# ylsung/vl-merging

Measured on AMD Instinct MI355X. Metric: VL samples/sec (fwd+bwd) base_vl 384^2 at 1/2/4/8 GPUs; merge GB/s vs HBM peak, higher is better.
Workload: dtype bf16

## Files before the change

### vl-merging_amd/csrc/rowops.hip

```cpp
#include "vlm_common.h"

#ifndef ROW_NT
#define ROW_NT true
#endif
#define ROW_THREADS 256
#define ROW_WAVES 4

template <int MAXU, bool IN_BF16, bool NT = false>
__device__ __forceinline__ void load_row(const void* base, size_t row, int ld, int D, int lane, f32x4 (&v)[MAXU]) {
#pragma unroll
  for (int u = 0; u < MAXU; ++u) {
    const int c = lane * 4 + 256 * u;
    if (c < D) {
      if (IN_BF16) {
        const bf16x4* q = reinterpret_cast<const bf16x4*>(reinterpret_cast<const bf16_t*>(base) + row * ld + c);
        const bf16x4 h = NT ? __builtin_nontemporal_load(q) : *q;
        v[u] = (f32x4){(float)h[0], (float)h[1], (float)h[2], (float)h[3]};
      } else {
        const f32x4* q = reinterpret_cast<const f32x4*>(reinterpret_cast<const float*>(base) + row * ld + c);
        v[u] = NT ? __builtin_nontemporal_load(q) : *q;
      }
    } else {
      v[u] = (f32x4){0.f, 0.f, 0.f, 0.f};
    }
  }
}

template <int MAXU>
__device__ __forceinline__ void load_vec(const float* p, int D, int lane, f32x4 (&v)[MAXU], float fill) {
#pragma unroll
  for (int u = 0; u < MAXU; ++u) {
    const int c = lane * 4 + 256 * u;
    v[u] = (c < D && p) ? *reinterpret_cast<const f32x4*>(p + c) : (f32x4){fill, fill, fill, fill};
// ... 35 lines not shown
    if (stats && lane == 0) {
      stats[2 * row] = mean;
      stats[2 * row + 1] = rstd;
    }
#pragma unroll
    for (int u = 0; u < MAXU; ++u) {
      const int c = lane * 4 + 256 * u;
      if (c < D) {
        f32x4 o;
#pragma unroll
        for (int r = 0; r < 4; ++r) o[r] = (v[u][r] - mean) * rstd * g[u][r] + b[u][r];
        if (OUT_F32) {
          *reinterpret_cast<f32x4*>(reinterpret_cast<float*>(y) + row * ldy + c) = o;
        } else {
          bf16x4 h = {(bf16_t)o[0], (bf16_t)o[1], (bf16_t)o[2], (bf16_t)o[3]};
          *reinterpret_cast<bf16x4*>(reinterpret_cast<bf16_t*>(y) + row * ldy + c) = h;
        }
      }
    }
  }
}

struct ls_t {
  const bf16_t* y;
  int ldy;
  const float* gamma;
  const float* row_scale;
  bf16_t* dy;
  int lddy;
  float* dgamma;
  float* dbias;
  float* partials;
};
template <int MAXU, bool DY_BF16, int SCALE = 0>
__global__ __launch_bounds__(ROW_THREADS, MAXU <= 3 ? (SCALE ? 3 : 4) : 2) void ln_bwd_kernel(const void* __restrict__ dy, int lddy,
                                                             const float* __restrict__ x, int ldx,
                                                             const float* __restrict__ stats,
                                                             const float* __restrict__ gamma, int M, int D,
                                                             const float* __restrict__ dres, int lddres,
                                                             float* __restrict__ dx, int lddx,
                                                             float* __restrict__ dgamma, float* __restrict__ dbeta,
                                                             float* __restrict__ partials, const ls_t ls) {
  __shared__ float red[ROW_WAVES][SCALE ? 4 : 2][MAXU * 256];
  const int lane = threadIdx.x & 63, wave = threadIdx.x >> 6;
  f32x4 g[SCALE ? 1 : MAXU], ag[MAXU], ab[MAXU];
  f32x4 g2[1], ag2[SCALE == 1 ? MAXU : 1], ab2[SCALE ? MAXU : 1];
  if (SCALE) g[0] = (f32x4){1.f, 1.f, 1.f, 1.f};
  else load_vec<SCALE ? 1 : MAXU>(gamma, D, lane, g, 1.0f);
#pragma unroll
  for (int u = 0; u < MAXU; ++u) ag[u] = ab[u] = (f32x4){0.f, 0.f, 0.f, 0.f};
#pragma unroll
  for (int u = 0; u < (SCALE ? MAXU : 1); ++u) ab2[u] = (f32x4){0.f, 0.f, 0.f, 0.f};
#pragma unroll
  for (int u = 0; u < (SCALE == 1 ? MAXU : 1); ++u) ag2[u] = (f32x4){0.f, 0.f, 0.f, 0.f};
  const float invD = 1.0f / (float)D;
  for (size_t row = (size_t)blockIdx.x * ROW_WAVES + wave; row < (size_t)M; row += (size_t)gridDim.x * ROW_WAVES) {
    f32x4 v[MAXU], d[MAXU], rs[MAXU];
    load_row<MAXU, false, ROW_NT>(x, row, ldx, D, lane, v);
    load_row<MAXU, DY_BF16>(dy, row, lddy, D, lane, d);
    if (dres) load_row<MAXU, false, ROW_NT>(dres, row, lddres, D, lane, rs);
    f32x4 yy[SCALE == 1 ? MAXU : 1];
    float srow = 1.0f;
    if (SCALE) {
      if (SCALE == 1) load_row<SCALE == 1 ? MAXU : 1, true, ROW_NT>(ls.y, row, ls.ldy, D, lane, yy);
      if (ls.row_scale) srow = ls.row_scale[row];
    }
    const float mean = stats[2 * row], rstd = stats[2 * row + 1];
    float s1 = 0.f, s2 = 0.f;
#pragma unroll
    for (int u = 0; u < MAXU; ++u) {
      const int c = lane * 4 + 256 * u;
      if (c < D) {
        const f32x4 gu = (SCALE && gamma) ? *reinterpret_cast<const f32x4*>(gamma + c) : g[SCALE ? 0 : u];
#pragma unroll
        for (int r = 0; r < 4; ++r) {
          const float xh = (v[u][r] - mean) * rstd;
          const float gg = d[u][r] * gu[r];
          s1 += gg;
          s2 += gg * xh;
          ag[u][r] += d[u][r] * xh;
          ab[u][r] += d[u][r];
          v[u][r] = xh;
          d[u][r] = gg;
        }
      }
    }
    const float m1 = wave_sum(s1) * invD, m2 = wave_sum(s2) * invD;
#pragma unroll
    for (int u = 0; u < MAXU; ++u) {
      const int c = lane * 4 + 256 * u;
      if (c < D) {
        f32x4 o;
#pragma unroll
        for (int r = 0; r < 4; ++r) o[r] = rstd * (d[u][r] - m1 - v[u][r] * m2);
        if (dres) o += rs[u];
        *reinterpret_cast<f32x4*>(dx + row * lddx + c) = o;
        if (SCALE) {
          const int c2 = lane * 4 + 256 * u;
          g2[0] = (SCALE == 1 && ls.gamma) ? *reinterpret_cast<const f32x4*>(ls.gamma + c2) : (f32x4){1.f, 1.f, 1.f, 1.f};
          bf16x4 h;
#pragma unroll
          for (int r = 0; r < 4; ++r) {
            const float sd = srow * o[r];
            const float q = sd * g2[0][r];
            if (SCALE == 1) ag2[SCALE == 1 ? u : 0][r] += sd * yy[SCALE == 1 ? u : 0][r];
            h[r] = (bf16_t)q;
            ab2[u][r] += (float)h[r];
          }
          *reinterpret_cast<bf16x4*>(ls.dy + row * ls.lddy + c) = h;
        }
      }
    }
  }
  if (SCALE) {
#pragma unroll
    for (int u = 0; u < (SCALE ? MAXU : 1); ++u)
#pragma unroll
      for (int r = 0; r < 4; ++r) {
        red[wave][SCALE ? 2 : 0][u * 256 + lane * 4 + r] = SCALE == 1 ? ag2[SCALE == 1 ? u : 0][r] : 0.f;
        red[wave][SCALE ? 3 : 1][u * 256 + lane * 4 + r] = ab2[u][r];
      }
  }
  if (dgamma || dbeta || SCALE) {
#pragma unroll
    for (int u = 0; u < MAXU; ++u)
#pragma unroll
      for (int r = 0; r < 4; ++r) {
        red[wave][0][u * 256 + lane * 4 + r] = ag[u][r];
        red[wave][1][u * 256 + lane * 4 + r] = ab[u][r];
      }
    __syncthreads();
    for (int c = threadIdx.x; c < D; c += ROW_THREADS) {
      float sg = 0.f, sb = 0.f;
#pragma unroll
      for (int w = 0; w < ROW_WAVES; ++w) {
        sg += red[w][0][c];
        sb += red[w][1][c];
      }
      if (partials) {
        partials[((size_t)blockIdx.x * 2 + 0) * D + c] = sg;
        partials[((size_t)blockIdx.x * 2 + 1) * D + c] = sb;
      } else {
        if (dgamma) atomicAdd(dgamma + c, sg);
        if (dbeta) atomicAdd(dbeta + c, sb);
      }
      if (SCALE) {
        float tg = 0.f, tb = 0.f;
#pragma unroll
        for (int w = 0; w < ROW_WAVES; ++w) {
          tg += red[w][SCALE ? 2 : 0][c];
          tb += red[w][SCALE ? 3 : 1][c];
        }
        if (ls.partials) {
          ls.partials[((size_t)blockIdx.x * 2 + 0) * D + c] = tg;
          ls.partials[((size_t)blockIdx.x * 2 + 1) * D + c] = tb;
        } else {
          if (ls.dgamma) atomicAdd(ls.dgamma + c, tg);
          if (ls.dbias) atomicAdd(ls.dbias + c, tb);
        }
      }
    }
  }
}

__global__ __launch_bounds__(256) void colreduce_kernel(const float* __restrict__ partials, int nblocks, int D,
                                                        float* __restrict__ out0, float* __restrict__ out1) {
  const int i = blockIdx.x * 256 + threadIdx.x;
  if (i >= 2 * D) return;
  const int which = i / D, c = i - which * D;
  float* out = which ? out1 : out0;
  if (!out) return;
  const int per = (nblocks + gridDim.y - 1) / gridDim.y;
  const int b0 = blockIdx.y * per, b1 = min(nblocks, b0 + per);
  float s0 = 0.f, s1 = 0.f;
  int b = b0;
  for (; b + 1 < b1; b += 2) {
    s0 += partials[((size_t)(b + 0) * 2 + which) * D + c];
    s1 += partials[((size_t)(b + 1) * 2 + which) * D + c];
  }
  if (b < b1) s0 += partials[((size_t)b * 2 + which) * D + c];
  if (b0 < b1) atomicAdd(out + c, s0 + s1);
}

struct fold_jobs_t {
  vlm_fold_job_t j[VLM_MAX_FOLD_JOBS];
};
__global__ __launch_bounds__(256) void colreduce_batch_kernel(const fold_jobs_t jobs) {
  const vlm_fold_job_t job = jobs.j[blockIdx.z];
  const int D = job.D, i = blockIdx.x * 256 + threadIdx.x;
  if (i >= 2 * D) return;
  const int which = i / D, c = i - which * D;
  float* out = which ? job.out1 : job.out0;
  if (!out) return;
  const int per = (job.nblocks + gridDim.y - 1) / gridDim.y;
// ... 117 lines not shown
  int want = (M + ROW_WAVES - 1) / ROW_WAVES;
  int cap = cus * 8;
  return want < cap ? (want > 0 ? want : 1) : cap;
}

extern "C" int vlm_layernorm_fwd(const float* x, int ldx, int M, int D, const float* gamma, const float* beta,
                                 float eps, void* y, int ldy, int y_is_f32, float* stats, void* stream) {
  if (M == 0) return VLM_OK;
  if (!x || !y || M < 0 || D <= 0 || (D & 3) || (ldx & 3) || (ldy & 3)) return VLM_ERR_ARG;
  if (D > 1024) return VLM_ERR_UNSUPPORTED;
  dim3 grid(row_grid(M)), block(ROW_THREADS);
  hipStream_t s = (hipStream_t)stream;
#define LN_FWD(U, F) hipLaunchKernelGGL((ln_fwd_kernel<U, F>), grid, block, 0, s, x, ldx, M, D, gamma, beta, eps, y, ldy, stats)
  if (D <= 256) { if (y_is_f32) LN_FWD(1, true); else LN_FWD(1, false); }
  else if (D <= 768) { if (y_is_f32) LN_FWD(3, true); else LN_FWD(3, false); }
  else { if (y_is_f32) LN_FWD(4, true); else LN_FWD(4, false); }
#undef LN_FWD
  VLM_CHECK_LAUNCH();
  return VLM_OK;
}

static int layernorm_bwd_impl(const void* dy, int lddy, int dy_is_f32, const float* x, int ldx,
                              const float* stats, const float* gamma, int M, int D, const float* dres,
                              int lddres, float* dx, int lddx, float* dgamma, float* dbeta, float* workspace,
                              size_t workspace_bytes, int* deferred_blocks, void* stream, const vlm_layerscale_t* sc) {
  if (M == 0) return VLM_OK;
  if (!dy || !x || !stats || !dx || M < 0 || D <= 0 || (D & 3) || (ldx & 3) || (lddy & 3) || (lddx & 3) ||
      (dres && (lddres & 3)))
    return VLM_ERR_ARG;
  if (D > 1024) return VLM_ERR_UNSUPPORTED;
  int g = row_grid(M);
  const int resident = (D <= 768 ? 4 : 2) * (vlm_device_cus() > 0 ? vlm_device_cus() : 256);
  if (g > resident) g = resident;
  if (sc && D <= 768 && g > resident * 3 / 4) g = resident * 3 / 4;
  float* part = (workspace && workspace_bytes >= (size_t)g * 2 * D * sizeof(float) && (dgamma || dbeta)) ? workspace : nullptr;
  dim3 grid(g), block(ROW_THREADS);
  hipStream_t s = (hipStream_t)stream;
  ls_t ls = {};
  if (sc) {
    if (!sc->dy || (sc->y && (sc->ldy & 3)) || (sc->lddy & 3)) return VLM_ERR_ARG;
    if (!sc->y && (sc->gamma || sc->dgamma)) return VLM_ERR_ARG;
    const bool want = sc->dgamma || sc->dbias;
    float* part2 = (sc->workspace && sc->workspace_bytes >= (size_t)g * 2 * D * sizeof(float) && want) ? sc->workspace : nullptr;
    if (deferred_blocks && want && !part2) return VLM_ERR_ARG;
    ls.y = reinterpret_cast<const bf16_t*>(sc->y); ls.ldy = sc->ldy; ls.gamma = sc->gamma; ls.row_scale = sc->row_scale;
    ls.dy = reinterpret_cast<bf16_t*>(sc->dy); ls.lddy = sc->lddy; ls.dgamma = sc->dgamma; ls.dbias = sc->dbias; ls.partials = part2;
  }
#define LN_BWD(U, B)                                                                                                             \
  do {                                                                                                                           \
    if (sc && sc->y) hipLaunchKernelGGL((ln_bwd_kernel<U, B, 1>), grid, block, 0, s, dy, lddy, x, ldx, stats, gamma, M, D, dres, lddres, dx, lddx, dgamma, dbeta, part, ls); \
    else if (sc) hipLaunchKernelGGL((ln_bwd_kernel<U, B, 2>), grid, block, 0, s, dy, lddy, x, ldx, stats, gamma, M, D, dres, lddres, dx, lddx, dgamma, dbeta, part, ls); \
    else hipLaunchKernelGGL((ln_bwd_kernel<U, B, 0>), grid, block, 0, s, dy, lddy, x, ldx, stats, gamma, M, D, dres, lddres, dx, lddx, dgamma, dbeta, part, ls); \
  } while (0)
  if (D <= 256) { if (dy_is_f32) LN_BWD(1, false); else LN_BWD(1, true); }
  else if (D <= 768) { if (dy_is_f32) LN_BWD(3, false); else LN_BWD(3, true); }
  else { if (dy_is_f32) LN_BWD(4, false); else LN_BWD(4, true); }
#undef LN_BWD
  VLM_CHECK_LAUNCH();
  if (deferred_blocks) {
    if (!part && (dgamma || dbeta)) return VLM_ERR_ARG;
    *deferred_blocks = (part || ls.partials) ? g : 0;
  } else {
    if (part) {
      hipLaunchKernelGGL(colreduce_kernel, dim3((2 * D + 255) / 256, 32), dim3(256), 0, s, part, g, D, dgamma, dbeta);
      VLM_CHECK_LAUNCH();
    }
    if (ls.partials) {
      hipLaunchKernelGGL(colreduce_kernel, dim3((2 * D + 255) / 256, 32), dim3(256), 0, s, ls.partials, g, D, ls.dgamma, ls.dbias);
      VLM_CHECK_LAUNCH();
    }
  }
  return VLM_OK;
}

extern "C" int vlm_layernorm_bwd(const void* dy, int lddy, int dy_is_f32, const float* x, int ldx,
                                 const float* stats, const float* gamma, int M, int D, const float* dres,
                                 int lddres, float* dx, int lddx, float* dgamma, float* dbeta, float* workspace,
                                 size_t workspace_bytes, int* deferred_blocks, void* stream) {
  return layernorm_bwd_impl(dy, lddy, dy_is_f32, x, ldx, stats, gamma, M, D, dres, lddres, dx, lddx, dgamma, dbeta, workspace,
                            workspace_bytes, deferred_blocks, stream, nullptr);
}

extern "C" int vlm_layernorm_bwd_scale(const void* dy, int lddy, int dy_is_f32, const float* x, int ldx,
                                       const float* stats, const float* gamma, int M, int D, const float* dres,
                                       int lddres, float* dx, int lddx, float* dgamma, float* dbeta, float* workspace,
// ... 53 lines not shown
```

### vl-merging_amd/engine.py

```python
import itertools
import math
import os
import weakref
from typing import List, Optional

import torch

from . import _lib as L
from . import ops

BF16, F32 = torch.bfloat16, torch.float32
ALIGN = 64


def _touch_hook(p):
    p._vlm_flat.touched.add(p._vlm_name)


def touch(*params):
    for p in params:
        if p is not None:
            f = getattr(p, "_vlm_flat", None)
            if f is not None:
                f.touched.add(p._vlm_name)
# ... 488 lines not shown


def _fb(b):
    return b._vlm_folded if b is not None else None


def _rb(b):
    return b._vlm_raw if b is not None else None


def _arm_layerscale_finish(flat):
    if getattr(flat, "_ls_armed", False):
        return
    flat._ls_armed = True

    def done():
        flat._ls_armed = False
        flat.finish_layerscale()
        sync_wgrad()

    torch.autograd.Variable._execution_engine.queue_callback(done)


def _ln2_bwd_scale1(dln, x1, st2, e, dx1, dx2, y1, g1, rs1, dy1, fold):
    sgamma, dsgamma, dsbias = (None, None, _rb(e.projb)) if y1 is None else (g1, g1.grad, e.projb.grad)
    if x1.shape[1] <= 768:
        ops.layernorm_bwd_scale(dln, x1, st2, e.n2w, dx1, dx2, e.n2w.grad, e.n2b.grad, y=y1, sgamma=sgamma, row_scale=rs1,
                                sdy=dy1, dsgamma=dsgamma, dsbias=dsbias, fold=fold)
    else:
        ops.layernorm_bwd(dln, x1, st2, e.n2w, dx1, dres=dx2, dgamma=e.n2w.grad, dbeta=e.n2b.grad, fold=fold)
        ops.layerscale_bwd(dx1, y1, sgamma, rs1, dy1, dsgamma, dsbias, fold=fold)


class _BlockFn(torch.autograd.Function):

    @staticmethod
    def forward(ctx, x, bias_t, plan: BlockPlan, pc: PassCtx, training: bool, hook):
        M, D = x.shape
        dev = x.device
        H = pc.H
        Fdim = plan.ranges[0][2].fc1w.shape[0]
        x = x.contiguous()
        ln1 = torch.empty(M, D, device=dev, dtype=BF16)
        st1 = torch.empty(M, 2, device=dev, dtype=F32)
        qkv = torch.empty(M, 3 * D, device=dev, dtype=BF16)
        rs1 = pc.drop_path_rows(plan.drop_prob, training, dev)
        rs2 = pc.drop_path_rows(plan.drop_prob, training, dev)
        rg = plan.ranges
        for r0, r1, e in rg:
            ops.layernorm_fwd(x[r0:r1], e.n1w, e.n1b, plan.eps, ln1[r0:r1], st1[r0:r1])
        _gemm_rows(ln1, [(r0, r1, w16(e.qkvw), _qkv_bias(e), None) for r0, r1, e in rg], qkv)
        o = torch.empty(M, D, device=dev, dtype=BF16)
        lse = torch.empty(H, M, device=dev, dtype=F32)
        rp = pc.relpos
        ops.attention_fwd(qkv, o, lse, pc.seq, H, bias_t=bias_t, head_row0=plan.layer * H,
                          rel_index=rp.index if rp is not None else None,
                          rel_index_t=rp.index_t if rp is not None else None, keep0=pc.keep0, keep1=pc.keep1,
                          mode=plan.mode, bias_dense=rp.dense_for(pc.seq, plan.mode) if rp is not None else None)
        x1 = torch.empty(M, D, device=dev, dtype=F32)
        folded = _folded(plan.ranges)
        y1 = torch.empty(M, D, device=dev, dtype=BF16) if not folded else None
        ln2 = torch.empty(M, D, device=dev, dtype=BF16)
        st2 = torch.empty(M, 2, device=dev, dtype=F32)
        h = torch.empty(M, Fdim, device=dev, dtype=BF16)
        a = torch.empty(M, Fdim, device=dev, dtype=BF16)
        x2 = torch.empty(M, D, device=dev, dtype=F32)
        y2 = torch.empty(M, D, device=dev, dtype=BF16) if not folded else None
        cs1, cs2 = (None, None) if folded else (plan.gamma1, plan.gamma2)
        pb = (lambda e: _fb(e.projb)) if folded else (lambda e: e.projb)
        fb2 = (lambda e: _fb(e.fc2b)) if folded else (lambda e: e.fc2b)
        _gemm_rows(o, [(r0, r1, w16(e.projw), pb(e), None) for r0, r1, e in rg], x1, col_scale=cs1, row_scale=rs1,
                   residual=x, aux=y1)
        for r0, r1, e in rg:
            ops.layernorm_fwd(x1[r0:r1], e.n2w, e.n2b, plan.eps, ln2[r0:r1], st2[r0:r1])
        _gemm_rows(ln2, [(r0, r1, w16(e.fc1w), e.fc1b, None) for r0, r1, e in rg], a, act=L.ACT_GELU_DERIV, aux=h)
        _gemm_rows(a, [(r0, r1, w16(e.fc2w), fb2(e), None) for r0, r1, e in rg], x2, col_scale=cs2, row_scale=rs2,
                   residual=x1, aux=y2)
        if pc.gram is not None:
            for r0, r1, e in plan.ranges:
                gn = e.gram_names
                if gn.get("qkv") or gn.get("fc1"):
                    t32 = torch.empty(r1 - r0, D, device=dev, dtype=F32)
                    st = torch.empty(r1 - r0, 2, device=dev, dtype=F32)
                    if gn.get("qkv"):
                        ops.layernorm_fwd(x[r0:r1], e.n1w, e.n1b, plan.eps, t32, st)
                        pc.gram.add(gn.get("qkv"), t32)
                    if gn.get("fc1"):
                        ops.layernorm_fwd(x1[r0:r1], e.n2w, e.n2b, plan.eps, t32, st)
                        pc.gram.add(gn.get("fc1"), t32)
                pc.gram.add(gn.get("proj"), o[r0:r1])
                pc.gram.add(gn.get("fc2"), a[r0:r1])
        ctx.plan, ctx.pc, ctx.hook = plan, pc, hook
        ctx.has_bias = bias_t is not None
        ctx.folded = folded
        ctx.save_for_backward(x, st1, ln1, qkv, o, lse, y1 if y1 is not None else x.new_empty(0), x1, st2, ln2, h, a,
                              y2 if y2 is not None else x.new_empty(0),
                              rs1 if rs1 is not None else x.new_empty(0), rs2 if rs2 is not None else x.new_empty(0),
                              bias_t if bias_t is not None else x.new_empty(0))
        return x2

    @staticmethod
    def backward(ctx, dx2):
        plan, pc = ctx.plan, ctx.pc
        x, st1, ln1, qkv, o, lse, y1, x1, st2, ln2, h, a, y2, rs1, rs2, bias_t = ctx.saved_tensors
        rs1 = rs1 if rs1.numel() else None
        rs2 = rs2 if rs2.numel() else None
        bias_t = bias_t if ctx.has_bias else None
        M, D = x.shape
        dev = x.device
        H = pc.H
        Fdim = h.shape[1]
        dx2 = dx2.contiguous()
        g1, g2 = plan.gamma1, plan.gamma2
        folded = ctx.folded
        if folded:
            y1 = y2 = None
            flat = plan.ranges[0][2].projw._vlm_flat
            _arm_layerscale_finish(flat)
        wg = (lambda w: w._vlm_raw) if folded else (lambda w: w.grad)
        touch(g1, g2)
        for _, _, e in plan.ranges:
            _touch_expert(e)
        dy2 = torch.empty(M, D, device=dev, dtype=BF16)
        dy1 = torch.empty(M, D, device=dev, dtype=BF16)
        dh = torch.empty(M, Fdim, device=dev, dtype=BF16)
        dln = torch.empty(M, D, device=dev, dtype=BF16)
        dx1 = torch.empty(M, D, device=dev, dtype=F32)
        fold = ops.FoldBatch(dev, D)
        rg = plan.ranges
        do = torch.empty(M, D, device=dev, dtype=BF16)
        for r0, r1, e in rg:
            rr = slice(r0, r1)
            if folded:
                ops.layerscale_bwd(dx2[rr], None, None, rs2[rr] if rs2 is not None else None, dy2[rr], None, _rb(e.fc2b), fold=fold)
            else:
                ops.layerscale_bwd(dx2[rr], y2[rr], g2, rs2[rr] if rs2 is not None else None, dy2[rr], g2.grad, e.fc2b.grad,
                                   fold=fold)
        _gemm_rows(dy2, [(r0, r1, wT16(e.fc2w), None, e.fc1b.grad) for r0, r1, e in rg], dh, act=L.ACT_MUL_AUX, aux=h,
                   col_sum_fold=fold)
        with _Side(dy2, a, dh, ln2):
            _wgrad_rows(dy2, a, [(r0, r1, wg(e.fc2w)) for r0, r1, e in rg])
            _wgrad_rows(dh, ln2, [(r0, r1, e.fc1w.grad) for r0, r1, e in rg])
        _gemm_rows(dh, [(r0, r1, wT16(e.fc1w), None, None) for r0, r1, e in rg], dln)
        for r0, r1, e in rg:
            rr = slice(r0, r1)
            _ln2_bwd_scale1(dln[rr], x1[rr], st2[rr], e, dx1[rr], dx2[rr], y1[rr] if y1 is not None else None, g1,
                            rs1[rr] if rs1 is not None else None, dy1[rr], fold)
        _gemm_rows(dy1, [(r0, r1, wT16(e.projw), None, None) for r0, r1, e in rg], do)
        with _Side(dy1, o):
            _wgrad_rows(dy1, o, [(r0, r1, wg(e.projw)) for r0, r1, e in rg])
        dqkv = torch.empty(M, 3 * D, device=dev, dtype=BF16)
        dln1 = torch.empty(M, D, device=dev, dtype=BF16)
        rp = pc.relpos
        qb_grads, vb_grads, fused_qv = _segment_bias_grads(rg, pc.seq)
        ops.attention_bwd(qkv, o, do, lse, dqkv, pc.seq, H, bias_t=bias_t, head_row0=plan.layer * H,
                          rel_index=rp.index if rp is not None else None,
                          rel_index_t=rp.index_t if rp is not None else None, keep0=pc.keep0, keep1=pc.keep1,
                          mode=plan.mode, dbias_t=rp.holder.get("dbias_t") if rp is not None else None,
                          dq_colsum=qb_grads, dv_colsum=vb_grads,
                          bias_dense=rp.dense_for(pc.seq, plan.mode) if rp is not None else None)
        dx = torch.empty(M, D, device=dev, dtype=F32)
        for r0, r1, e in rg:
            if e.qb is not None and not fused_qv:
                ops.colsum(dqkv[r0:r1, :D], e.qb.grad)
                ops.colsum(dqkv[r0:r1, 2 * D:], e.vb.grad)
        with _Side(dqkv, ln1):
            _wgrad_rows(dqkv, ln1, [(r0, r1, e.qkvw.grad) for r0, r1, e in rg])
        _gemm_rows(dqkv, [(r0, r1, wT16(e.qkvw), None, None) for r0, r1, e in rg], dln1)
        for r0, r1, e in rg:
            rr = slice(r0, r1)
            ops.layernorm_bwd(dln1[rr], x[rr], st1[rr], e.n1w, dx[rr], dres=dx1[rr], dgamma=e.n1w.grad, dbeta=e.n1b.grad,
                              fold=fold)
        fold.flush()
        if folded:
            flat.ls_pending.add(plan.layer)
        if ctx.hook is not None:
            ctx.hook(plan.layer)
        dbias = None
        if bias_t is not None and ctx.needs_input_grad[1] and rp is not None and not rp.holder.get("routed"):
            rp.holder["routed"] = True
            dbias = _zero_scalar(dev).expand_as(bias_t)
        return dx, dbias, None, None, None, None


def run_block(x, plan: BlockPlan, pc: PassCtx, training: bool, hook=None):
    bias_t = pc.relpos.bias_t if pc.relpos is not None else None
    return _BlockFn.apply(x, bias_t, plan, pc, training, hook)


class _LinearFn(torch.autograd.Function):

    @staticmethod
    def forward(ctx, x, weight, bias, act):
        x2 = x.reshape(-1, x.shape[-1])
        if x2.dtype != BF16:
            x2 = x2.to(BF16)
        if x2.stride(1) != 1 or (x2.shape[0] > 1 and x2.stride(0) < x2.shape[1]):
            x2 = x2.contiguous()
        M, K = x2.shape
        N = weight.shape[0]
        Np = (N + 63) // 64 * 64
        gelu = act == "gelu"
        buf = torch.empty(M, Np, device=x.device, dtype=BF16)
        pre = torch.empty(M, Np, device=x.device, dtype=BF16) if gelu else None
        ops.gemm(x2, w16(weight), buf[:, :N], bias=bias, act=L.ACT_GELU if gelu else L.ACT_NONE,
                 aux=pre[:, :N] if gelu else None)
        y = ops.tanh_fwd(buf[:, :N]) if act == "tanh" else None
        ctx.save_for_backward(x2, pre if gelu else (y if y is not None else x2.new_empty(0)))
        ctx.weight, ctx.bias, ctx.act, ctx.shape, ctx.N, ctx.Np = weight, bias, act, x.shape, N, Np
        return (y if y is not None else buf[:, :N]).view(*x.shape[:-1], N)

    @staticmethod
    def backward(ctx, gy):
        x2, saved = ctx.saved_tensors
        weight, bias, N, Np, act = ctx.weight, ctx.bias, ctx.N, ctx.Np, ctx.act
        M, K = x2.shape
        gy2 = gy.reshape(M, N)
        if gy2.dtype not in (BF16, F32):
            gy2 = gy2.float()
        if gy2.stride(1) != 1:
# ... 442 lines not shown
```

### vl-merging_amd/ops.py

```python
import ctypes

import torch

from . import _lib as L

BF16 = torch.bfloat16
F32 = torch.float32


def _ld(t):
    if t.dim() != 2 or t.stride(1) != 1:
        raise L.VlmError("expected a 2-D tensor with unit inner stride, got shape %s strides %s"
                         % (tuple(t.shape), t.stride()))
    return t.stride(0) if t.shape[0] > 1 else max(t.stride(0), t.shape[1])


def gemm(a, b, out, ta=False, tb=False, *, bias=None, act=L.ACT_NONE, aux=None, col_scale=None, row_scale=None,
         residual=None, alpha=1.0, accumulate=False, col_sum=None, col_sum_fold=None):
    L.require_cuda(a, b, out, bias, aux, col_scale, row_scale, residual, col_sum)
    if a.dtype != BF16 or b.dtype != BF16:
        raise L.VlmError("gemm operands must be bfloat16")
    M, N = out.shape
    K = a.shape[0] if ta else a.shape[1]
    if (a.shape[1] if ta else a.shape[0]) != M:
        raise L.VlmError("gemm: A rows %s do not match M=%d" % (tuple(a.shape), M))
    kb, nb = (b.shape[0], b.shape[1]) if tb else (b.shape[1], b.shape[0])
    if nb != N or kb != K:
        raise L.VlmError("gemm: B shape %s incompatible with N=%d K=%d" % (tuple(b.shape), N, K))
    e = L.Epilogue()
    e.bias = bias.data_ptr() if bias is not None else 0
    e.col_scale = col_scale.data_ptr() if col_scale is not None else 0
    e.row_scale = row_scale.data_ptr() if row_scale is not None else 0
# ... 99 lines not shown
        if ldc is not None and _ld(dW) != ldc:
            raise L.VlmError("gemm_wgrad_grouped: the groups' gradients must share one leading dimension")
        ldc = _ld(dW)
        prev = r1
        g.row0, g.rows, g.C, g.accumulate = r0, r1 - r0, dW.data_ptr(), int(bool(accumulate))
    ws = _splitk_workspace(dy.device)
    rc = L.get_lib().vlm_gemm_wgrad_grouped(len(groups), arr, M, N, L.ptr(dy), _ld(dy), L.ptr(x), _ld(x), ldc, L.ptr(ws),
                                            ws.numel() * 4, L.stream_ptr())
    L.check(rc, "vlm_gemm_wgrad_grouped")


_SPLITK_WS = {}
SPLITK_WS_BYTES = 96 << 20


def _splitk_workspace(device):
    key = (device.index, torch.cuda.current_stream().cuda_stream)
    ws = _SPLITK_WS.get(key)
    if ws is None:
        ws = _SPLITK_WS[key] = torch.empty(SPLITK_WS_BYTES // 4, device=device, dtype=F32)
    return ws


def layernorm_fwd(x, gamma, beta, eps, out, stats=None):
    L.require_cuda(x, gamma, beta, out, stats)
    M, D = x.shape
    rc = L.get_lib().vlm_layernorm_fwd(L.ptr(x), _ld(x), M, D, L.ptr(gamma), L.ptr(beta), eps, L.ptr(out), _ld(out),
                                       int(out.dtype == F32), L.ptr(stats), L.stream_ptr())
    L.check(rc, "vlm_layernorm_fwd")
    return out


_ROW_WS = {}


def _row_workspace(device, D, slot=0):
    key = (device.index, torch.cuda.current_stream().cuda_stream, slot)
    n = 1536 * 2 * max(D, 1024)
    ws = _ROW_WS.get(key)
    if ws is None or ws.numel() < n:
        ws = _ROW_WS[key] = torch.empty(n, device=device, dtype=F32)
    return ws


class FoldBatch:

    MAX = 16

    def __init__(self, device, D=1024):
        self.region = 1536 * 2 * max(D, 1024)
        key = ("fold", device.index, torch.cuda.current_stream().cuda_stream)
        ws = _ROW_WS.get(key)
        if ws is None or ws.numel() < self.MAX * self.region:
            ws = _ROW_WS[key] = torch.empty(self.MAX * self.region, device=device, dtype=F32)
        self.ws = ws
        self.jobs = []
        self.taken = 0

    def next_region(self):
        return self.next_regions(1)[0]

    def next_regions(self, n):
        if self.taken + n > self.MAX:
            self.flush()
        i = self.taken
        self.taken += n
        return [self.ws[(i + k) * self.region:(i + k + 1) * self.region] for k in range(n)]

    def add(self, region, nblocks, D, out0, out1):
        if nblocks > 0:
            self.jobs.append((region, nblocks, D, out0, out1))

    def flush(self):
        self.taken = 0
        if not self.jobs:
            return
        arr = (L.FoldJob * len(self.jobs))()
        for a, (region, nblocks, D, out0, out1) in zip(arr, self.jobs):
            a.partials, a.nblocks, a.D = region.data_ptr(), nblocks, D
            a.out0 = out0.data_ptr() if out0 is not None else None
            a.out1 = out1.data_ptr() if out1 is not None else None
        L.check(L.get_lib().vlm_colreduce_batch(arr, len(self.jobs), L.stream_ptr()), "vlm_colreduce_batch")
        self.jobs = []


def layernorm_bwd(dy, x, stats, gamma, dx, dres=None, dgamma=None, dbeta=None, fold=None):
    L.require_cuda(dy, x, stats, gamma, dx, dres, dgamma, dbeta)
    M, D = x.shape
    ws = fold.next_region() if fold is not None else _row_workspace(x.device, D)
    nb = ctypes.c_int(0)
    rc = L.get_lib().vlm_layernorm_bwd(L.ptr(dy), _ld(dy), int(dy.dtype == F32), L.ptr(x), _ld(x), L.ptr(stats),
                                       L.ptr(gamma), M, D, L.ptr(dres), _ld(dres) if dres is not None else 0,
                                       L.ptr(dx), _ld(dx), L.ptr(dgamma), L.ptr(dbeta), L.ptr(ws), ws.numel() * 4,
                                       ctypes.byref(nb) if fold is not None else None, L.stream_ptr())
    L.check(rc, "vlm_layernorm_bwd")
    if fold is not None:
        fold.add(ws, nb.value, D, dgamma, dbeta)
    return dx


def layernorm_bwd_scale(dy, x, stats, gamma, dx, dres, dgamma, dbeta, *, y, sgamma, row_scale, sdy, dsgamma=None, dsbias=None,
                        fold=None):
    L.require_cuda(dy, x, stats, gamma, dx, dres, dgamma, dbeta, y, sgamma, row_scale, sdy, dsgamma, dsbias)
    M, D = x.shape
    nb = ctypes.c_int(0)
    if fold is not None:
        ws, ws2 = fold.next_regions(2)
    else:
        ws, ws2 = _row_workspace(x.device, D), _row_workspace(x.device, D, slot=1)
    sc = L.LayerScale()
    sc.y, sc.ldy, sc.gamma, sc.row_scale = L.ptr(y), _ld(y) if y is not None else 0, L.ptr(sgamma), L.ptr(row_scale)
    sc.dy, sc.lddy, sc.dgamma, sc.dbias = L.ptr(sdy), _ld(sdy), L.ptr(dsgamma), L.ptr(dsbias)
    sc.workspace, sc.workspace_bytes = L.ptr(ws2), ws2.numel() * 4
    rc = L.get_lib().vlm_layernorm_bwd_scale(L.ptr(dy), _ld(dy), int(dy.dtype == F32), L.ptr(x), _ld(x), L.ptr(stats),
                                             L.ptr(gamma), M, D, L.ptr(dres), _ld(dres) if dres is not None else 0,
                                             L.ptr(dx), _ld(dx), L.ptr(dgamma), L.ptr(dbeta), L.ptr(ws), ws.numel() * 4,
                                             ctypes.byref(sc), ctypes.byref(nb) if fold is not None else None, L.stream_ptr())
    L.check(rc, "vlm_layernorm_bwd_scale")
    if fold is not None:
        fold.add(ws, nb.value if (dgamma is not None or dbeta is not None) else 0, D, dgamma, dbeta)
        fold.add(ws2, nb.value if (dsgamma is not None or dsbias is not None) else 0, D, dsgamma, dsbias)
    return dx


def layerscale_bwd(dx, y, gamma, row_scale, dy, dgamma=None, dbias=None, fold=None):
    L.require_cuda(dx, y, gamma, row_scale, dy, dgamma, dbias)
    M, D = dx.shape
    ws = fold.next_region() if fold is not None else _row_workspace(dx.device, D)
    nb = ctypes.c_int(0)
    rc = L.get_lib().vlm_layerscale_bwd(L.ptr(dx), _ld(dx), L.ptr(y), _ld(y) if y is not None else 0, L.ptr(gamma), L.ptr(row_scale), M, D,
                                        L.ptr(dy), _ld(dy), L.ptr(dgamma), L.ptr(dbias), L.ptr(ws), ws.numel() * 4,
                                        ctypes.byref(nb) if fold is not None else None, L.stream_ptr())
    L.check(rc, "vlm_layerscale_bwd")
    if fold is not None:
        fold.add(ws, nb.value, D, dgamma, dbias)
    return dy


def embedding_bwd(gy, ids, dW, padding_idx=-1):
    L.require_cuda(gy, ids, dW)
    n, D = gy.shape
    assert gy.dtype == F32 and dW.dtype == F32 and ids.dtype == torch.int64 and ids.numel() == n and gy.stride(1) == 1
    L.check(L.get_lib().vlm_embedding_bwd(L.ptr(gy), _ld(gy), L.ptr(ids), n, D, int(padding_idx), L.ptr(dW), _ld(dW),
                                          dW.shape[0], L.stream_ptr()), "vlm_embedding_bwd")
    return dW


def cross_entropy_fwd(logits, labels, ignore_index=-100):
    L.require_cuda(logits, labels)
    rows, V = logits.shape
    if logits.dtype != BF16 or labels.dtype != torch.int64 or labels.numel() != rows or not labels.is_contiguous():
        raise L.VlmError("cross_entropy: bf16 logits [rows, V], contiguous int64 labels [rows]")
    loss_rows = torch.empty(rows, device=logits.device, dtype=F32)
    lse = torch.empty(rows, device=logits.device, dtype=F32)
    L.check(L.get_lib().vlm_cross_entropy_fwd(L.ptr(logits), _ld(logits), rows, V, L.ptr(labels), int(ignore_index), L.ptr(loss_rows),
                                              L.ptr(lse), L.stream_ptr()), "vlm_cross_entropy_fwd")
    return loss_rows, lse


def cross_entropy_bwd(logits, labels, lse, scale, ignore_index=-100):
    L.require_cuda(logits, labels, lse, scale)
    rows, V = logits.shape
    Vp = (V + 63) // 64 * 64
    buf = torch.empty(rows, Vp, device=logits.device, dtype=BF16)
    L.check(L.get_lib().vlm_cross_entropy_bwd(L.ptr(logits), _ld(logits), rows, V, L.ptr(labels), int(ignore_index), L.ptr(lse),
                                              L.ptr(scale), L.ptr(buf), Vp, L.stream_ptr()), "vlm_cross_entropy_bwd")
# ... 609 lines not shown
```

### vl-merging_amd/vilt/modules/vision_transformer.py

```python
import math

import torch
import torch.nn as nn

from ... import _lib as L
from ... import engine
from ... import ops


def trunc_normal_(t, std=0.02):
    return nn.init.trunc_normal_(t, mean=0.0, std=std, a=-2.0, b=2.0)


class Mlp(nn.Module):
    def __init__(self, in_features, hidden_features=None, out_features=None):
        super().__init__()
        self.fc1 = nn.Linear(in_features, hidden_features or in_features)
        self.fc2 = nn.Linear(hidden_features or in_features, out_features or in_features)


class Attention(nn.Module):
    def __init__(self, dim, num_heads=8, qkv_bias=False, qk_scale=None):
        super().__init__()
        self.num_heads = num_heads
# ... 107 lines not shown
                ranges = []
                if seq.n0:
                    ranges.append((rows0[0], rows0[1], self._expert("l")))
                if seq.n1:
                    ranges.append((rows1[0], rows1[1], self._expert("v")))
        elif type_id == 0:
            ranges = [(lo, hi, self._expert("v"))]
        elif type_id == 1:
            ranges = [(lo, hi, self._expert("l"))]
        elif self.tasks is not None and "vl" in self.tasks:
            ranges = [(lo, hi, self._expert("vl"))]
        elif not any_dict and not self.separate_inference:
            ranges = [(lo, hi, self._expert("vl"))]
        else:
            if isinstance(self.attn, nn.ModuleDict):
                if not self.self_attn_for_single_mode:
                    raise NotImplementedError("in_attn MoE with self_attn_for_single_mode=False (both experts over "
                                              "all tokens, vision_transformer.py:641-651) is not on the hot path")
                mode = L.ATTN_SEPARATE
            else:
                mode = L.ATTN_SEPARATE if self.separate_inference else L.ATTN_JOINT
            if any_dict:
                ranges = []
                if seq.n0:
                    ranges.append((rows0[0], rows0[1], self._expert("l")))
                if seq.n1:
                    ranges.append((rows1[0], rows1[1], self._expert("v")))
            else:
                ranges = [(lo, hi, self._expert("v"))]
        p = engine.BlockPlan(ranges, mode, self.gamma_1, self.gamma_2, self.layer_number, self.drop_path_prob, self.eps)
        self._plans[k] = p
        return p

    def run(self, x, pc, type_id, hook=None):
        return engine.run_block(x, self.plan(type_id, pc.seq), pc, self.training, hook)

    def forward(self, x, mask=None, type_id=None, relative_position_bias=None):
        B, N, D = x.shape
        if type_id == 0:
            n0, n1 = 0, N
        elif type_id == 1:
            n0, n1 = N, 0
        else:
            n0, n1 = self.max_text_len, N - self.max_text_len
        seq = ops.Seq(B, n0, n1)
        rows = torch.cat([x[:, :n0].reshape(B * n0, D), x[:, n0:].reshape(B * n1, D)], 0).float()
        keep0 = keep1 = None
        if mask is not None:
            mk = mask.to(torch.uint8)
            keep0 = mk[:, :n0].contiguous() if n0 else None
            keep1 = mk[:, n0:].contiguous() if n1 else None
        pc = engine.PassCtx(seq, self.num_heads, relative_position_bias, keep0, keep1)
        y = self.run(rows, pc, 2 if type_id is None else type_id)
        out = torch.cat([y[:B * n0].view(B, n0, D), y[B * n0:].view(B, n1, D)], 1)
        return out, None


class PatchEmbed(nn.Module):
    def __init__(self, img_size=224, patch_size=16, in_chans=3, embed_dim=768):
        super().__init__()
        self.img_size = (img_size, img_size)
        self.patch_size = (patch_size, patch_size)
        self.patch_shape = (img_size // patch_size, img_size // patch_size)
        self.num_patches = self.patch_shape[0] * self.patch_shape[1]
        self.proj = nn.Conv2d(in_chans, embed_dim, kernel_size=patch_size, stride=patch_size)

    def forward(self, x):
        return engine.patch_embed(x, self.proj.weight, self.proj.bias, self.patch_size[0])
# ... 72 lines not shown
```

Baseline: 338.6.

## Fuse next block's LayerScale backward into previous block's LayerNorm backward

Adds a cross-block handoff so that the backward pass of a block computes the layer below's LayerScale/residual backward (dy2 and its bias/gamma partials) inside the LN1 backward kernel. The lower block then reuses the precomputed dy2 and skips its own layerscale_bwd pass over dx2. A dedicated cast kernel handles the folded (no y) case without the unused gamma-gradient accumulator. The goal is to remove one full read/write pass over the residual gradient per block. In exchange it adds fragile bookkeeping (workspace slot ownership, tensor version checks) and a Python call counter.

```diff
diff --git a/vl-merging_amd/csrc/rowops.hip b/vl-merging_amd/csrc/rowops.hip
--- a/vl-merging_amd/csrc/rowops.hip
+++ b/vl-merging_amd/csrc/rowops.hip
@@ -1,4 +1,6 @@
 #include "vlm_common.h"
+
+#include <type_traits>
 
 #ifndef ROW_NT
 #define ROW_NT true
@@ -100,7 +102,7 @@
   float* dbias;
   float* partials;
 };
-template <int MAXU, bool DY_BF16, int SCALE = 0>
+template <int MAXU, bool DY_BF16, bool SCALE = false>
 __global__ __launch_bounds__(ROW_THREADS, MAXU <= 3 ? (SCALE ? 3 : 4) : 2) void ln_bwd_kernel(const void* __restrict__ dy, int lddy,
                                                              const float* __restrict__ x, int ldx,
                                                              const float* __restrict__ stats,
@@ -112,7 +114,7 @@
   __shared__ float red[ROW_WAVES][SCALE ? 4 : 2][MAXU * 256];
   const int lane = threadIdx.x & 63, wave = threadIdx.x >> 6;
   f32x4 g[SCALE ? 1 : MAXU], ag[MAXU], ab[MAXU];
-  f32x4 g2[1], ag2[SCALE == 1 ? MAXU : 1], ab2[SCALE ? MAXU : 1];
+  f32x4 g2[1], ag2[SCALE ? MAXU : 1], ab2[SCALE ? MAXU : 1];
   if (SCALE) g[0] = (f32x4){1.f, 1.f, 1.f, 1.f};
   else load_vec<SCALE ? 1 : MAXU>(gamma, D, lane, g, 1.0f);
 #pragma unroll
@@ -120,17 +122,17 @@
 #pragma unroll
   for (int u = 0; u < (SCALE ? MAXU : 1); ++u) ab2[u] = (f32x4){0.f, 0.f, 0.f, 0.f};
 #pragma unroll
-  for (int u = 0; u < (SCALE == 1 ? MAXU : 1); ++u) ag2[u] = (f32x4){0.f, 0.f, 0.f, 0.f};
+  for (int u = 0; u < (SCALE ? MAXU : 1); ++u) ag2[u] = (f32x4){0.f, 0.f, 0.f, 0.f};
   const float invD = 1.0f / (float)D;
   for (size_t row = (size_t)blockIdx.x * ROW_WAVES + wave; row < (size_t)M; row += (size_t)gridDim.x * ROW_WAVES) {
     f32x4 v[MAXU], d[MAXU], rs[MAXU];
     load_row<MAXU, false, ROW_NT>(x, row, ldx, D, lane, v);
     load_row<MAXU, DY_BF16>(dy, row, lddy, D, lane, d);
     if (dres) load_row<MAXU, false, ROW_NT>(dres, row, lddres, D, lane, rs);
-    f32x4 yy[SCALE == 1 ? MAXU : 1];
+    f32x4 yy[SCALE ? MAXU : 1];
     float srow = 1.0f;
     if (SCALE) {
-      if (SCALE == 1) load_row<SCALE == 1 ? MAXU : 1, true, ROW_NT>(ls.y, row, ls.ldy, D, lane, yy);
+      load_row<SCALE ? MAXU : 1, true, ROW_NT>(ls.y, row, ls.ldy, D, lane, yy);
       if (ls.row_scale) srow = ls.row_scale[row];
     }
     const float mean = stats[2 * row], rstd = stats[2 * row + 1];
@@ -165,13 +167,13 @@
         *reinterpret_cast<f32x4*>(dx + row * lddx + c) = o;
         if (SCALE) {
           const int c2 = lane * 4 + 256 * u;
-          g2[0] = (SCALE == 1 && ls.gamma) ? *reinterpret_cast<const f32x4*>(ls.gamma + c2) : (f32x4){1.f, 1.f, 1.f, 1.f};
+          g2[0] = ls.gamma ? *reinterpret_cast<const f32x4*>(ls.gamma + c2) : (f32x4){1.f, 1.f, 1.f, 1.f};
           bf16x4 h;
 #pragma unroll
           for (int r = 0; r < 4; ++r) {
             const float sd = srow * o[r];
             const float q = sd * g2[0][r];
-            if (SCALE == 1) ag2[SCALE == 1 ? u : 0][r] += sd * yy[SCALE == 1 ? u : 0][r];
+            ag2[SCALE ? u : 0][r] += sd * yy[SCALE ? u : 0][r];
             h[r] = (bf16_t)q;
             ab2[u][r] += (float)h[r];
           }
@@ -185,7 +187,7 @@
     for (int u = 0; u < (SCALE ? MAXU : 1); ++u)
 #pragma unroll
       for (int r = 0; r < 4; ++r) {
-        red[wave][SCALE ? 2 : 0][u * 256 + lane * 4 + r] = SCALE == 1 ? ag2[SCALE == 1 ? u : 0][r] : 0.f;
+        red[wave][SCALE ? 2 : 0][u * 256 + lane * 4 + r] = ag2[SCALE ? u : 0][r];
         red[wave][SCALE ? 3 : 1][u * 256 + lane * 4 + r] = ab2[u][r];
       }
   }
@@ -228,6 +230,105 @@
         }
       }
     }
+  }
+}
+
+template <int MAXU, bool DY_BF16>
+__global__ __launch_bounds__(ROW_THREADS, MAXU <= 3 ? 4 : 2) void ln_bwd_cast_kernel(const void* __restrict__ dy, int lddy,
+                                                             const float* __restrict__ x, int ldx,
+                                                             const float* __restrict__ stats,
+                                                             const float* __restrict__ gamma, int M, int D,
+                                                             const float* __restrict__ dres, int lddres,
+                                                             float* __restrict__ dx, int lddx,
+                                                             float* __restrict__ dgamma, float* __restrict__ dbeta,
+                                                             float* __restrict__ partials, const ls_t ls) {
+  __shared__ float red[ROW_WAVES][3][MAXU * 256];
+  const int lane = threadIdx.x & 63, wave = threadIdx.x >> 6;
+  using raw_t = typename std::conditional<DY_BF16, bf16x4, f32x4>::type;
+  f32x4 ag[MAXU], ab[MAXU], ab2[MAXU];
+#pragma unroll
+  for (int u = 0; u < MAXU; ++u) ag[u] = ab[u] = ab2[u] = (f32x4){0.f, 0.f, 0.f, 0.f};
+  const float invD = 1.0f / (float)D;
+  for (size_t row = (size_t)blockIdx.x * ROW_WAVES + wave; row < (size_t)M; row += (size_t)gridDim.x * ROW_WAVES) {
+    f32x4 v[MAXU], rs[MAXU];
+    raw_t d[MAXU];
+    load_row<MAXU, false, ROW_NT>(x, row, ldx, D, lane, v);
+#pragma unroll
+    for (int u = 0; u < MAXU; ++u) {
+      const int c = lane * 4 + 256 * u;
+      if (c < D) d[u] = *reinterpret_cast<const raw_t*>(DY_BF16 ? (const void*)(reinterpret_cast<const bf16_t*>(dy) + row * lddy + c)
+                                                                 : (const void*)(reinterpret_cast<const float*>(dy) + row * lddy + c));
+    }
+    if (dres) load_row<MAXU, false, ROW_NT>(dres, row, lddres, D, lane, rs);
+    const float srow = ls.row_scale ? ls.row_scale[row] : 1.0f;
+    const float mean = stats[2 * row], rstd = stats[2 * row + 1];
+    float s1 = 0.f, s2 = 0.f;
+#pragma unroll
+    for (int u = 0; u < MAXU; ++u) {
+      const int c = lane * 4 + 256 * u;
+      if (c < D) {
+        const f32x4 gu = gamma ? *reinterpret_cast<const f32x4*>(gamma + c) : (f32x4){1.f, 1.f, 1.f, 1.f};
+#pragma unroll
+        for (int r = 0; r < 4; ++r) {
+          const float xh = (v[u][r] - mean) * rstd;
+          const float dd = (float)d[u][r];
+          const float gg = dd * gu[r];
+          s1 += gg;
+          s2 += gg * xh;
+          ag[u][r] += dd * xh;
+          v[u][r] = xh;
+        }
+      }
+    }
+    const float m1 = wave_sum(s1) * invD, m2 = wave_sum(s2) * invD;
+#pragma unroll
+    for (int u = 0; u < MAXU; ++u) {
+      const int c = lane * 4 + 256 * u;
+      if (c < D) {
+        const f32x4 gu = gamma ? *reinterpret_cast<const f32x4*>(gamma + c) : (f32x4){1.f, 1.f, 1.f, 1.f};
+        f32x4 o;
+        bf16x4 h;
+#pragma unroll
+        for (int r = 0; r < 4; ++r) {
+          const float dd = (float)d[u][r];
+          ab[u][r] += dd;
+          o[r] = rstd * (dd * gu[r] - m1 - v[u][r] * m2);
+        }
+        if (dres) o += rs[u];
+        *reinterpret_cast<f32x4*>(dx + row * lddx + c) = o;
+#pragma unroll
+        for (int r = 0; r < 4; ++r) {
+          h[r] = (bf16_t)(srow * o[r]);
+          ab2[u][r] += (float)h[r];
+        }
+        *reinterpret_cast<bf16x4*>(ls.dy + row * ls.lddy + c) = h;
+      }
+    }
+  }
+#pragma unroll
+  for (int u = 0; u < MAXU; ++u) {
+    *reinterpret_cast<f32x4*>(&red[wave][0][u * 256 + lane * 4]) = ag[u];
+    *reinterpret_cast<f32x4*>(&red[wave][1][u * 256 + lane * 4]) = ab[u];
+    *reinterpret_cast<f32x4*>(&red[wave][2][u * 256 + lane * 4]) = ab2[u];
+  }
+  __syncthreads();
+  for (int c = threadIdx.x; c < D; c += ROW_THREADS) {
+    float sg = 0.f, sb = 0.f, tb = 0.f;
+#pragma unroll
+    for (int w = 0; w < ROW_WAVES; ++w) {
+      sg += red[w][0][c];
+      sb += red[w][1][c];
+      tb += red[w][2][c];
+    }
+    if (partials) {
+      partials[((size_t)blockIdx.x * 2 + 0) * D + c] = sg;
+      partials[((size_t)blockIdx.x * 2 + 1) * D + c] = sb;
+    } else {
+      if (dgamma) atomicAdd(dgamma + c, sg);
+      if (dbeta) atomicAdd(dbeta + c, sb);
+    }
+    if (ls.partials) ls.partials[((size_t)blockIdx.x * 2 + 1) * D + c] = tb;
+    else if (ls.dbias) atomicAdd(ls.dbias + c, tb);
   }
 }
 
@@ -411,7 +512,7 @@
   int g = row_grid(M);
   const int resident = (D <= 768 ? 4 : 2) * (vlm_device_cus() > 0 ? vlm_device_cus() : 256);
   if (g > resident) g = resident;
-  if (sc && D <= 768 && g > resident * 3 / 4) g = resident * 3 / 4;
+  if (sc && sc->y && D <= 768 && g > resident * 3 / 4) g = resident * 3 / 4;
   float* part = (workspace && workspace_bytes >= (size_t)g * 2 * D * sizeof(float) && (dgamma || dbeta)) ? workspace : nullptr;
   dim3 grid(g), block(ROW_THREADS);
   hipStream_t s = (hipStream_t)stream;
@@ -427,9 +528,9 @@
   }
 #define LN_BWD(U, B)                                                                                                             \
   do {                                                                                                                           \
-    if (sc && sc->y) hipLaunchKernelGGL((ln_bwd_kernel<U, B, 1>), grid, block, 0, s, dy, lddy, x, ldx, stats, gamma, M, D, dres, lddres, dx, lddx, dgamma, dbeta, part, ls); \
-    else if (sc) hipLaunchKernelGGL((ln_bwd_kernel<U, B, 2>), grid, block, 0, s, dy, lddy, x, ldx, stats, gamma, M, D, dres, lddres, dx, lddx, dgamma, dbeta, part, ls); \
-    else hipLaunchKernelGGL((ln_bwd_kernel<U, B, 0>), grid, block, 0, s, dy, lddy, x, ldx, stats, gamma, M, D, dres, lddres, dx, lddx, dgamma, dbeta, part, ls); \
+    if (sc && sc->y) hipLaunchKernelGGL((ln_bwd_kernel<U, B, true>), grid, block, 0, s, dy, lddy, x, ldx, stats, gamma, M, D, dres, lddres, dx, lddx, dgamma, dbeta, part, ls); \
+    else if (sc) hipLaunchKernelGGL((ln_bwd_cast_kernel<U, B>), grid, block, 0, s, dy, lddy, x, ldx, stats, gamma, M, D, dres, lddres, dx, lddx, dgamma, dbeta, part, ls); \
+    else hipLaunchKernelGGL((ln_bwd_kernel<U, B, false>), grid, block, 0, s, dy, lddy, x, ldx, stats, gamma, M, D, dres, lddres, dx, lddx, dgamma, dbeta, part, ls); \
   } while (0)
   if (D <= 256) { if (dy_is_f32) LN_BWD(1, false); else LN_BWD(1, true); }
   else if (D <= 768) { if (dy_is_f32) LN_BWD(3, false); else LN_BWD(3, true); }
diff --git a/vl-merging_amd/engine.py b/vl-merging_amd/engine.py
--- a/vl-merging_amd/engine.py
+++ b/vl-merging_amd/engine.py
@@ -544,10 +544,47 @@
         ops.layerscale_bwd(dx1, y1, sgamma, rs1, dy1, dsgamma, dsbias, fold=fold)
 
 
+class _Handoff:
+
+    __slots__ = ("pc", "plan", "folded", "rs2", "y2", "consumers", "dx", "dx_version", "dy2", "jobs", "slots")
+
+    def __init__(self, pc, plan):
+        self.pc, self.plan = pc, plan
+        self.folded, self.rs2, self.y2 = False, None, None
+        self.consumers = 0
+        self.dx = self.dy2 = self.jobs = self.slots = None
+        self.dx_version = -1
+
+    def release(self):
+        self.rs2 = self.y2 = self.dx = self.dy2 = self.jobs = None
+
+
+_HANDOFF_OWNER = {}
+
+
+def _handoff_regions(dev, D, reg, n):
+    stream = torch.cuda.current_stream().cuda_stream
+    out = []
+    for i in range(n):
+        slot = 2 + 2 * (reg.plan.layer & 1) + i
+        _HANDOFF_OWNER[(dev.index, stream, slot)] = reg
+        out.append(ops._row_workspace(dev, D, slot=slot))
+    reg.slots = [(dev.index, stream, 2 + 2 * (reg.plan.layer & 1) + i) for i in range(n)]
+    return out
+
+
+def _handoff_applies(rg, below, M, D):
+    if below is None or below.consumers != 1 or below.dy2 is not None or D > 768 or len(rg) > 2:
+        return False
+    rb = below.plan.ranges
+    return len(rb) == len(rg) and all(a[0] == b[0] and a[1] == b[1] for a, b in zip(rg, rb)) and \
+        (below.rs2 is None or below.rs2.shape[0] >= M)
+
+
 class _BlockFn(torch.autograd.Function):
 
     @staticmethod
-    def forward(ctx, x, bias_t, plan: BlockPlan, pc: PassCtx, training: bool, hook):
+    def forward(ctx, x, bias_t, plan: BlockPlan, pc: PassCtx, training: bool, hook, below=None, reg=None):
         M, D = x.shape
         dev = x.device
         H = pc.H
@@ -603,6 +640,9 @@
                 pc.gram.add(gn.get("proj"), o[r0:r1])
                 pc.gram.add(gn.get("fc2"), a[r0:r1])
         ctx.plan, ctx.pc, ctx.hook = plan, pc, hook
+        ctx.below, ctx.reg = below, reg
+        if reg is not None:
+            reg.folded, reg.rs2, reg.y2 = folded, rs2, y2
         ctx.has_bias = bias_t is not None
         ctx.folded = folded
         ctx.save_for_backward(x, st1, ln1, qkv, o, lse, y1 if y1 is not None else x.new_empty(0), x1, st2, ln2, h, a,
@@ -622,6 +662,11 @@
         dev = x.device
         H = pc.H
         Fdim = h.shape[1]
+        reg, took = ctx.reg, False
+        if reg is not None and reg.dy2 is not None:
+            took = (dx2.data_ptr() == reg.dx.data_ptr() and dx2.shape == reg.dx.shape and dx2.dtype == F32 and
+                    dx2.is_contiguous() and dx2._version == reg.dx_version and
+                    all(_HANDOFF_OWNER.get(k) is reg for k in reg.slots))
         dx2 = dx2.contiguous()
         g1, g2 = plan.gamma1, plan.gamma2
         folded = ctx.folded
@@ -633,7 +678,7 @@
         touch(g1, g2)
         for _, _, e in plan.ranges:
             _touch_expert(e)
-        dy2 = torch.empty(M, D, device=dev, dtype=BF16)
+        dy2 = reg.dy2 if took else torch.empty(M, D, device=dev, dtype=BF16)
         dy1 = torch.empty(M, D, device=dev, dtype=BF16)
         dh = torch.empty(M, Fdim, device=dev, dtype=BF16)
         dln = torch.empty(M, D, device=dev, dtype=BF16)
@@ -641,7 +686,15 @@
         fold = ops.FoldBatch(dev, D)
         rg = plan.ranges
         do = torch.empty(M, D, device=dev, dtype=BF16)
-        for r0, r1, e in rg:
+        if took:
+            for job in reg.jobs:
+                fold.add(*job)
+        if reg is not None:
+            for k in (reg.slots or ()):
+                if _HANDOFF_OWNER.get(k) is reg:
+                    del _HANDOFF_OWNER[k]
+            reg.release()
+        for r0, r1, e in (() if took else rg):
             rr = slice(r0, r1)
             if folded:
                 ops.layerscale_bwd(dx2[rr], None, None, rs2[rr] if rs2 is not None else None, dy2[rr], None, _rb(e.fc2b), fold=fold)
@@ -679,10 +732,24 @@
         with _Side(dqkv, ln1):
             _wgrad_rows(dqkv, ln1, [(r0, r1, e.qkvw.grad) for r0, r1, e in rg])
         _gemm_rows(dqkv, [(r0, r1, wT16(e.qkvw), None, None) for r0, r1, e in rg], dln1)
-        for r0, r1, e in rg:
-            rr = slice(r0, r1)
-            ops.layernorm_bwd(dln1[rr], x[rr], st1[rr], e.n1w, dx[rr], dres=dx1[rr], dgamma=e.n1w.grad, dbeta=e.n1b.grad,
-                              fold=fold)
+        below = ctx.below
+        if _handoff_applies(rg, below, M, D):
+            below.dy2 = torch.empty(M, D, device=dev, dtype=BF16)
+            below.jobs = []
+            g2b = below.plan.gamma2
+            for (r0, r1, e), (_, _, eb), region in zip(rg, below.plan.ranges, _handoff_regions(dev, D, below, len(rg))):
+                rr = slice(r0, r1)
+                y, sg, dsg, dsb = (None, None, None, _rb(eb.fc2b)) if below.folded else (below.y2[rr], g2b, g2b.grad, eb.fc2b.grad)
+                ops.layernorm_bwd_scale(dln1[rr], x[rr], st1[rr], e.n1w, dx[rr], dx1[rr], e.n1w.grad, e.n1b.grad, y=y, sgamma=sg,
+                                        row_scale=below.rs2[rr] if below.rs2 is not None else None, sdy=below.dy2[rr],
+                                        dsgamma=dsg, dsbias=dsb, fold=fold, park=(region, below.jobs))
+            below.dx, below.dx_version = dx, dx._version
+        else:
+            for r0, r1, e in rg:
+                rr = slice(r0, r1)
+                ops.layernorm_bwd(dln1[rr], x[rr], st1[rr], e.n1w, dx[rr], dres=dx1[rr], dgamma=e.n1w.grad, dbeta=e.n1b.grad,
+                                  fold=fold)
+        ctx.below = None
         fold.flush()
         if folded:
             flat.ls_pending.add(plan.layer)
@@ -692,12 +759,23 @@
         if bias_t is not None and ctx.needs_input_grad[1] and rp is not None and not rp.holder.get("routed"):
             rp.holder["routed"] = True
             dbias = _zero_scalar(dev).expand_as(bias_t)
-        return dx, dbias, None, None, None, None
-
-
-def run_block(x, plan: BlockPlan, pc: PassCtx, training: bool, hook=None):
+        return dx, dbias, None, None, None, None, None, None
+
+
+def run_block(x, plan: BlockPlan, pc: PassCtx, training: bool, hook=None, handoff=True):
     bias_t = pc.relpos.bias_t if pc.relpos is not None else None
-    return _BlockFn.apply(x, bias_t, plan, pc, training, hook)
+    below = getattr(x, "_vlm_handoff", None)
+    if below is not None:
+        below.consumers += 1
+        if not handoff or below.pc is not pc:
+            below = None
+    reg = None
+    if handoff and pc.gram is None and torch.is_grad_enabled() and x.shape[1] <= 768:
+        reg = _Handoff(pc, plan)
+    out = _BlockFn.apply(x, bias_t, plan, pc, training, hook, below, reg)
+    if reg is not None:
+        out._vlm_handoff = reg
+    return out
 
 
 class _LinearFn(torch.autograd.Function):
diff --git a/vl-merging_amd/ops.py b/vl-merging_amd/ops.py
--- a/vl-merging_amd/ops.py
+++ b/vl-merging_amd/ops.py
@@ -1,3 +1,4 @@
+import collections
 import ctypes
 
 import torch
@@ -163,6 +164,7 @@
 
 
 _ROW_WS = {}
+CALLS = collections.Counter()
 
 
 def _row_workspace(device, D, slot=0):
@@ -212,6 +214,7 @@
             a.out0 = out0.data_ptr() if out0 is not None else None
             a.out1 = out1.data_ptr() if out1 is not None else None
         L.check(L.get_lib().vlm_colreduce_batch(arr, len(self.jobs), L.stream_ptr()), "vlm_colreduce_batch")
+        CALLS["colreduce_batch"] += 1
         self.jobs = []
 
 
@@ -225,17 +228,22 @@
                                        L.ptr(dx), _ld(dx), L.ptr(dgamma), L.ptr(dbeta), L.ptr(ws), ws.numel() * 4,
                                        ctypes.byref(nb) if fold is not None else None, L.stream_ptr())
     L.check(rc, "vlm_layernorm_bwd")
+    CALLS["layernorm_bwd"] += 1
     if fold is not None:
         fold.add(ws, nb.value, D, dgamma, dbeta)
     return dx
 
 
 def layernorm_bwd_scale(dy, x, stats, gamma, dx, dres, dgamma, dbeta, *, y, sgamma, row_scale, sdy, dsgamma=None, dsbias=None,
-                        fold=None):
+                        fold=None, park=None):
     L.require_cuda(dy, x, stats, gamma, dx, dres, dgamma, dbeta, y, sgamma, row_scale, sdy, dsgamma, dsbias)
     M, D = x.shape
     nb = ctypes.c_int(0)
-    if fold is not None:
+    if park is not None:
+        if fold is None:
+            raise L.VlmError("layernorm_bwd_scale: park= defers the LayerScale's fold, which needs fold=")
+        ws, ws2 = fold.next_region(), park[0]
+    elif fold is not None:
         ws, ws2 = fold.next_regions(2)
     else:
         ws, ws2 = _row_workspace(x.device, D), _row_workspace(x.device, D, slot=1)
@@ -248,9 +256,14 @@
                                              L.ptr(dx), _ld(dx), L.ptr(dgamma), L.ptr(dbeta), L.ptr(ws), ws.numel() * 4,
                                              ctypes.byref(sc), ctypes.byref(nb) if fold is not None else None, L.stream_ptr())
     L.check(rc, "vlm_layernorm_bwd_scale")
+    CALLS["layernorm_bwd_scale"] += 1
     if fold is not None:
         fold.add(ws, nb.value if (dgamma is not None or dbeta is not None) else 0, D, dgamma, dbeta)
-        fold.add(ws2, nb.value if (dsgamma is not None or dsbias is not None) else 0, D, dsgamma, dsbias)
+        job = (ws2, nb.value if (dsgamma is not None or dsbias is not None) else 0, D, dsgamma, dsbias)
+        if park is not None:
+            park[1].append(job)
+        else:
+            fold.add(*job)
     return dx
 
 
@@ -263,6 +276,7 @@
                                         L.ptr(dy), _ld(dy), L.ptr(dgamma), L.ptr(dbias), L.ptr(ws), ws.numel() * 4,
                                         ctypes.byref(nb) if fold is not None else None, L.stream_ptr())
     L.check(rc, "vlm_layerscale_bwd")
+    CALLS["layerscale_bwd"] += 1
     if fold is not None:
         fold.add(ws, nb.value, D, dgamma, dbias)
     return dy
diff --git a/vl-merging_amd/vilt/modules/vision_transformer.py b/vl-merging_amd/vilt/modules/vision_transformer.py
--- a/vl-merging_amd/vilt/modules/vision_transformer.py
+++ b/vl-merging_amd/vilt/modules/vision_transformer.py
@@ -163,8 +163,8 @@
         self._plans[k] = p
         return p
 
-    def run(self, x, pc, type_id, hook=None):
-        return engine.run_block(x, self.plan(type_id, pc.seq), pc, self.training, hook)
+    def run(self, x, pc, type_id, hook=None, handoff=True):
+        return engine.run_block(x, self.plan(type_id, pc.seq), pc, self.training, hook, handoff=handoff)
 
     def forward(self, x, mask=None, type_id=None, relative_position_bias=None):
         B, N, D = x.shape
```

Measured after the change: 341.1 (median of 6 runs). Within noise of the previous version (+0.7%).
